# vibevoice-community/VibeVoice

Hardware: AMD Instinct MI355X
Metric: audio-sec/wall-sec (higher is better)
Workload: dtype bf16

## Files before the change

### vibevoice_amd/csrc/block1d.hip

```cpp
#include "vv_common.h"

namespace {

__device__ __forceinline__ float wsum(float v) {
#pragma unroll
    for (int o = 32; o > 0; o >>= 1) v += __shfl_xor(v, o);
    return v;
}
__device__ __forceinline__ float gelu_erf(float u) { return 0.5f * u * (1.0f + erff(u * 0.70710678118654752440f)); }

struct VVBlock {
    const float* xin;
    float* xout;
    float* nst;
    const float *norm_w, *ffn_norm_w, *gamma, *ffn_gamma, *dw_w , *dw_b, *b1, *b2;
    const u32x4 *w1, *w2;
    int T;
    float eps;
    VVSlotIds sl;
    int64_t sx, snst;
};

template <int XS>
__device__ __forceinline__ void split_store(unsigned char* base, size_t part_stride, int byte_off, float v) {
// ... 127 lines not shown
        xs[e] += gam_r * acc;
    }
    __syncthreads();
    for (int r = wave; r < TT; r += 4) {
        float s = 0.f;
        float xr[CL];
#pragma unroll
        for (int q = 0; q < CL; ++q) { const int c = lane + q * 64; xr[q] = (c < C) ? xs[r * C + c] : 0.f; s += xr[q] * xr[q]; }
        const float rr = rsqrtf(wsum(s) / (float)C + a.eps);
#pragma unroll
        for (int q = 0; q < CL; ++q) {
            const int c = lane + q * 64;
            if (c < C) {
                const float n = xr[q] * rr * fnw_r[q];
                const int off = (((c >> 5) * 64 + r + 16 * ((c & 31) >> 3)) * 8 + (c & 7)) * 2;
                split_store<XS>(f1, (size_t)KT1 * 1024, off, n);
            }
        }
    }
    __syncthreads();
#pragma unroll
    for (int i1 = 0; i1 < M1; ++i1) {
        const int nt = wave + 4 * i1;
        if (nt >= NT1) break;
        f32x4 acc = {0.f, 0.f, 0.f, 0.f};
#pragma unroll
        for (int kt = 0; kt < KT1; ++kt) {
            const bf16x8 wf = __builtin_bit_cast(bf16x8, w1r[i1][kt]);
#pragma unroll
            for (int p = 0; p < XS; ++p) {
                const bf16x8 xb = __builtin_bit_cast(bf16x8, *reinterpret_cast<const u32x4*>(f1 + ((size_t)(p * KT1 + kt) * 64 + lane) * 16));
                acc = __builtin_amdgcn_mfma_f32_16x16x32_bf16(wf, xb, acc, 0, 0, 0);
            }
        }
        const int n0 = nt * 16 + fq * 4;
        float u[4];
        const float bb[4] = {b1_r[i1].x, b1_r[i1].y, b1_r[i1].z, b1_r[i1].w};
#pragma unroll
        for (int r = 0; r < 4; ++r) u[r] = gelu_erf(acc[r] + bb[r]);
        const int off = (((n0 >> 5) * 64 + frow + 16 * ((n0 & 31) >> 3)) * 8 + (n0 & 7)) * 2;
#pragma unroll
        for (int r = 0; r < 4; ++r) split_store<XS>(f2, (size_t)KT2 * 1024, off + r * 2, u[r]);
    }
    __syncthreads();
#pragma unroll
    for (int i2 = 0; i2 < M2; ++i2) {
        const int nt = wave + 4 * i2;
        if (nt >= NT2) break;
        f32x4 acc = {0.f, 0.f, 0.f, 0.f};
#pragma unroll
        for (int kt = 0; kt < KT2; ++kt) {
            const bf16x8 wf = __builtin_bit_cast(bf16x8, w2r[i2][kt]);
#pragma unroll
            for (int p = 0; p < XS; ++p) {
                const bf16x8 ub = __builtin_bit_cast(bf16x8, *reinterpret_cast<const u32x4*>(f2 + ((size_t)(p * KT2 + kt) * 64 + lane) * 16));
                acc = __builtin_amdgcn_mfma_f32_16x16x32_bf16(wf, ub, acc, 0, 0, 0);
            }
        }
        const int c0 = nt * 16 + fq * 4;
        const int t = t0 + frow;
        if (t < a.T) {
            float4 o;
            o.x = xs[frow * C + c0 + 0] + fg_r[i2].x * (acc[0] + b2_r[i2].x);
            o.y = xs[frow * C + c0 + 1] + fg_r[i2].y * (acc[1] + b2_r[i2].y);
            o.z = xs[frow * C + c0 + 2] + fg_r[i2].z * (acc[2] + b2_r[i2].z);
            o.w = xs[frow * C + c0 + 3] + fg_r[i2].w * (acc[3] + b2_r[i2].w);
            *reinterpret_cast<float4*>(xout + (int64_t)t * C + c0) = o;
        }
    }
}

template <int C, int XS>
static void go(const VVBlock& a, hipStream_t s) {
    constexpr int TT = 16, HALO = 6, F = 4 * C;
    const size_t smem = (size_t)((TT + HALO) * C + TT * C + TT) * 4 + (size_t)XS * (C / 32) * 1024 + (size_t)XS * (F / 32) * 1024;
    static bool attr = false;
    if (!attr) {
        hipFuncSetAttribute(reinterpret_cast<const void*>(&vv_block1d_kernel<C, XS>), hipFuncAttributeMaxDynamicSharedMemorySize, 160 * 1024);
        attr = true;
    }
    hipLaunchKernelGGL((vv_block1d_kernel<C, XS>), dim3((a.T + TT - 1) / TT, a.sl.n > 0 ? a.sl.n : 1), dim3(256), smem, s, a);
}

}

extern "C" int vv_block1d_supported(int C) { return C == 32 || C == 64 || C == 128; }
extern "C" int vv_block1d_slots_launch(int C, int xs, const float* xin, float* xout, float* nst, const float* norm_w,
                                       const float* ffn_norm_w, const float* gamma, const float* ffn_gamma,
                                       const float* dw_w, const float* dw_b, const float* b1, const float* b2,
                                       const void* w1, const void* w2, int T, float eps, const int* ids, int n, int64_t sx,
                                       int64_t snst, hipStream_t s);

extern "C" int vv_block1d_launch(int C, int xs, const float* xin, float* xout, float* nst, const float* norm_w,
                                 const float* ffn_norm_w, const float* gamma, const float* ffn_gamma,
                                 const float* dw_w, const float* dw_b, const float* b1, const float* b2,
                                 const void* w1, const void* w2, int T, float eps, hipStream_t s) {
    return vv_block1d_slots_launch(C, xs, xin, xout, nst, norm_w, ffn_norm_w, gamma, ffn_gamma, dw_w, dw_b, b1, b2, w1, w2, T, eps,
                                   nullptr, 0, 0, 0, s);
}

extern "C" int vv_block1d_slots_launch(int C, int xs, const float* xin, float* xout, float* nst, const float* norm_w,
                                       const float* ffn_norm_w, const float* gamma, const float* ffn_gamma,
                                       const float* dw_w, const float* dw_b, const float* b1, const float* b2,
                                       const void* w1, const void* w2, int T, float eps, const int* ids, int n, int64_t sx,
                                       int64_t snst, hipStream_t s) {
    if (n < 0 || n > 8) return -1;
    VVBlock a{xin, xout, nst, norm_w, ffn_norm_w, gamma, ffn_gamma, dw_w, dw_b, b1, b2,
              (const u32x4*)w1, (const u32x4*)w2, T, eps};
    a.sl.n = ids ? n : 0;
    for (int i = 0; i < 8; ++i) a.sl.id[i] = (ids && i < n) ? ids[i] : 0;
    a.sx = sx; a.snst = snst;
#define VV_B(C_)                                                     \
    do {                                                             \
        if (xs == 1) go<C_, 1>(a, s);                                \
        else if (xs == 2) go<C_, 2>(a, s);                           \
        else go<C_, 3>(a, s);                                        \
    } while (0)
    if (C == 32) VV_B(32);
    else if (C == 64) VV_B(64);
    else if (C == 128) VV_B(128);
    else return -1;
#undef VV_B
    return vv_launch_rc(0);
}
```

### vibevoice_amd/csrc/engine.hip

```cpp
#include <algorithm>
#include <cmath>
#include <cstdarg>
#include <cstdio>
#include <cstdlib>
#include <cstring>
#include <functional>
#include <map>
#include <set>
#include <string>
#include <vector>

#include <mutex>
#include <shared_mutex>
#include "../../include/vvhip.h"
#include "vv_common.h"

extern "C" {
int vv_gemm_launch(VVGemm a, int xs, hipStream_t s);
int vv_pack_launch(const void* src, int src_is_bf16, void* dst, int N, int K, int kind, int Cin, int Cout, int ksz,
                   int stride, hipStream_t s);
int vv_rope_append_launch(int D, const float* qkv, const VVRow* rows, const float* inv_freq, float* q_out, void* kc,
                          void* vc, int R, int Hq, int Hkv, int64_t cache_stride, int64_t head_stride, hipStream_t s);
int vv_rope_table_launch(const float* inv_freq, void* tab, int n_pos, int half, hipStream_t s);
int vv_attn_fused_launch(int D, int xs, const float* qkv, const VVRow* rows, const void* rope_tab, void* kc, void* vc,
                         int R, int Hq, int Hkv, int64_t cache_stride, int64_t head_stride, int S,
                         float* pm, float* pl, float* po, float* out, void* out_packed, hipStream_t s);
int vv_attn_launch(int D, int xs, const float* q, const VVRow* rows, const void* kc, const void* vc, int R, int Hq,
                   int Hkv, int64_t cache_stride, int64_t head_stride, int S, float* pm, float* pl, float* po,
                   float* out, hipStream_t s);
int vv_embed_launch(const void* table, const int* ids, float* out, int n, int H, hipStream_t s);
int vv_logits_full_launch(const void* table, const float* hidden, float* out, int n, int V, int H, hipStream_t s);
int vv_rmsnorm_rows_launch(const float* x, int ldx, float* y, int ldy, const float* w, int T, int C, float eps, hipStream_t s);
int vv_dwconv_res_launch(const float* nb, const float* x, float* xo, const float* w, const float* b, const float* gamma, int T, int C, hipStream_t s);
int vv_normdw_sliced_ok(int T, int C);
int vv_normdw_sliced_launch(const float* xin, float* xout, float* nb, const float* nw, const float* w, const float* b,
                            const float* gamma, int T, int C, float eps, hipStream_t s);
int vv_normdw_sliced_slots_launch(const float* xin, float* xout, float* nb, const float* nw, const float* w, const float* b,
                                  const float* gamma, int T, int C, float eps, const int* ids, int n, int64_t sx, int64_t snb,
                                  hipStream_t s);
int vv_normdw_rows_slots_launch(const float* xin, float* xout, float* nb, const float* nw, const float* w, const float* b,
                                const float* gamma, int T, int C, float eps, const int* ids, int n, int64_t sx, int64_t snb,
                                hipStream_t s);
int vv_stem_conv_slots_launch(const float* in, const void* wp, const float* bias, float* out, int T, int N, const int* ids, int n,
                              int64_t s_in, int64_t s_out, hipStream_t s);
int vv_head_conv1_slots_launch(const float* x, const void* wp, const float* bias, float* out, int T, int Cin, const int* ids, int n,
                               int64_t s_in, int64_t s_out, hipStream_t s);
int vv_block1d_slots_launch(int C, int xs, const float* xin, float* xout, float* nst, const float* norm_w,
                            const float* ffn_norm_w, const float* gamma, const float* ffn_gamma,
                            const float* dw_w, const float* dw_b, const float* b1, const float* b2,
                            const void* w1, const void* w2, int T, float eps, const int* ids, int n, int64_t sx,
                            int64_t snst, hipStream_t s);
int vv_affine_slots_launch(const float* x, float* y, float mul, float add, int L, const int* ids, int n, int64_t stride, hipStream_t s);
int vv_normdw_launch(float* x, float* nb, const float* nw, const float* w, const float* b, const float* gamma, int T, int C,
                     float eps, hipStream_t s);
int vv_normdw_rows_ok(int T, int C);
int vv_normdw_rows_launch(const float* xin, float* xout, float* nb, const float* nw, const float* w, const float* b,
                          const float* gamma, int T, int C, float eps, hipStream_t s);
int vv_stem_conv_launch(const float* in, const void* wp, const float* bias, float* out, int T, int N, hipStream_t s);
int vv_head_conv1_launch(const float* x, const void* wp, const float* bias, float* out, int T, int Cin, hipStream_t s);
int vv_shift_rows_launch(const void* tab, int n_entries, int maxC, hipStream_t s);
int vv_zero_hist_launch(const void* tab, int n_entries, hipStream_t s);
int vv_cfg_dpm_launch(const float* eps, float* x, float* x0_prev, const float* coef, float cfg, int n, int L, const float* sde_noise, hipStream_t s);
int vv_affine_launch(const float* x, float* y, float mul, float add, int n, hipStream_t s);
int vv_copy_launch(void* dst, const void* src, size_t bytes, hipStream_t s);
int vv_zero_launch(void* dst, size_t bytes, hipStream_t s);
int vv_sampler_init_launch(const float* noise, float* z, float* x0p, int nL, hipStream_t s);
int vv_add_launch(const float* a, const float* b, float* y, int n, hipStream_t s);
int vv_tfreq_launch(const float* t, float* out, int n, hipStream_t s);
int vv_silu_launch(float* x, int n, hipStream_t s);
int vv_ada_in_launch(const float* cproj, const float* temb, float* out, int rows, int n_steps, int H, hipStream_t s);
int vv_add_rows_launch(const float* x, const float* v, float* y, int n, int C, hipStream_t s);
int vv_relu_launch(float* x, int n, hipStream_t s);
int vv_kv_import_launch(const void* k, const void* v, int src_bf16, void* kc, void* vc, int L, int Hkv, int D, int64_t head_stride, int pos0, hipStream_t s);
int vv_kv_move_launch(void* kc, void* vc, int layers, int Hkv, int D, int64_t layer_stride, int64_t head_stride, int src, int dst, hipStream_t s);
int vv_kv_zero_v_tail_launch(void* vc, const VVRow* rows, int R, int layers, int Hkv, int D, int64_t cache_stride, int64_t layer_stride,
                             int64_t head_stride, int max_ctx, hipStream_t s);
int vv_pcm16_launch(const float* x, short* out, int n, int samples, hipStream_t s);
int vv_cvt_launch(const void* src, void* dst, int64_t n, int to_bf16, hipStream_t s);
int vv_dw_transpose_launch(const float* src, float* dst, int C, hipStream_t s);
int vv_pack_rows_launch(const float* x, int ldx, const float* nw, float eps, void* xp, int T, int K, hipStream_t s);
int vv_unpack_rows_launch(const void* xp, float* x, int T, int K, hipStream_t s);
int vv_pack16_launch(const float* x, int ldx, int mode, const float* nw, float eps, const float* sc, const float* sh, int ld_mod,
                     void* xp, int T, int K, hipStream_t s);
int vv_gemv16p_launch(const void* W, const void* W2, const void* Xp, float* Y, void* Yp, const float* bias, const float* gate,
                      int T, int N, int K, int ldy, int ld_gate, int epi, hipStream_t s);
int vv_gemv16p_launch2(const VVGemv16p* a, int epi, int flags, hipStream_t s);
int vv_head_tail_ok(const VVTail* a);
int vv_head_tail_init();
int vv_head_tail_launch(const VVTail* a, hipStream_t s);
int vv_pack16_tiles_launch(const float* x, int ldx, int64_t stride_outer, int n_inner, int64_t stride_inner, void* xp, int64_t tile_bytes,
                           int T, int K, int n_tiles, hipStream_t s);
int vv_ada_pack_launch(const float* cproj, const float* temb, void* xp, int rows, int n_steps, int H, hipStream_t s);
int vv_gemm3_launch(const void* W, const void* W2, const void* Xp, float* Y, void* Yp, const float* bias, int T, int N, int K,
                    int ldy, int epi, const VVGemmWs* ws, hipStream_t s);
int vv_gemm_qkv_rope_launch(const void* W, const void* Xp, const float* bias, int T, int K, int D, int Hq, int Hkv, const VVRow* rows_dev,
                            const void* rope_tab, float* q_out, void* kc, void* vc, int64_t cache_stride, int64_t head_stride,
                            const VVGemmWs* ws, hipStream_t s);
int vv_attn_prefill4_launch(int D, const float* q, const VVRow* rows, const void* kc, const void* vc, int R, int Hq, int Hkv,
                            int64_t cache_stride, int64_t head_stride, float* out, void* out_packed, hipStream_t s);
int vv_block1d_supported(int C);
int vv_gemv_ok(const VVGemm* a);
int vv_tile_ok(const VVGemm* a, int xs);
int vv_block1d_launch(int C, int xs, const float* xin, float* xout, float* nst, const float* norm_w,
                      const float* ffn_norm_w, const float* gamma, const float* ffn_gamma, const float* dw_w,
                      const float* dw_b, const float* b1, const float* b2, const void* w1, const void* w2, int T,
                      float eps, hipStream_t s);
}

struct VVShiftH { float* buf; int T, hist, C; };

static thread_local char g_err[512] = "";
static std::shared_mutex g_dev_mu;
#define VV_SHARED std::shared_lock<std::shared_mutex> _vv_dev_lk(g_dev_mu)
static std::mutex g_family_mu;

namespace {

enum WKind { W_MAT = 0, W_VEC = 1, W_DW = 2, W_TABLE = 3, W_BIAS_REP = 4 };

struct Weight {
    std::string name;
    int kind = W_VEC;
    int64_t nelem = 0;
    void* dev = nullptr;
    int N = 0, K = 0, pk = 0, Cin = 0, Cout = 0, ksz = 0, stride = 0;
    int rep = 1;
    bool loaded = false;
    bool optional = false;
};

struct Block {
    int C;
    float *norm_w, *ffn_norm_w, *gamma, *ffn_gamma, *dw_w, *dw_b, *b1, *b2;
    void *w1, *w2;
    float* nb;
    float* nst;
    int64_t nb_stride;
};

struct ConvG {
    void* w; float* bias;
    int K, N, ldx;
    int rows_per_frame;
};

struct Stage {
    int C, Tpf;
    int hist;
    float* xs;
    float* xs2;
    float* xfinal;
    bool fused;
    bool pp;
    int64_t sl_stride;
    std::vector<Block> blocks;
    ConvG in;
};

struct CodecNet {
    bool decoder = false;
    int Fmax = 1, in_dim = 1, out_dim = 1, in_hist = 6, in_Tpf = 1;
    std::vector<float*> in_buf;
    std::vector<std::vector<Stage>> st;
    ConvG head;
    std::vector<float*> u;
    std::vector<std::map<int, void*>> shift_tab;
    std::vector<int> shift_n;
    std::vector<void*> zero_tab;
    int maxC = 1;
    int kd = 0, ke = 1 << 30;
    bool head_batch = false;
    int64_t in_stride = 0, u_stride = 0;
    std::map<uint64_t, std::pair<void*, int>> shift_multi;
};

struct GraphEntry { hipGraphExec_t exec; uint64_t last_use; };

}

struct vv_ctx {
    vv_config c;
    char err[512];
    std::vector<Weight> w;
// ... 366 lines not shown
    *tab_out = d; *n_out = (int)t.size();
    return 0;
}
static int codec_tables(vv_ctx* ctx, CodecNet& net, int sl, int F, void** tab_out, int* n_out) {
    auto it = net.shift_tab[sl].find(F);
    if (it != net.shift_tab[sl].end()) { *tab_out = it->second; *n_out = net.shift_n[sl]; return 0; }
    std::vector<VVShiftH> t;
    codec_table_entries(net, sl, F, t);
    void* d = dalloc(ctx, t.size() * sizeof(VVShiftH), false);
    if (!d) return -1;
    HIPCHK(ctx, hipMemcpy(d, t.data(), t.size() * sizeof(VVShiftH), hipMemcpyHostToDevice));
    net.shift_tab[sl][F] = d; net.shift_n[sl] = (int)t.size();
    *tab_out = d; *n_out = (int)t.size();
    return 0;
}

static VVGemm mk_gemm(const void* W, const float* X, float* Y, int T, int N, int K, int ldx, int ldy) {
    VVGemm g; memset(&g, 0, sizeof(g));
    g.W = (const u32x4*)W; g.X = X; g.Y = Y; g.T = T; g.N = N; g.K = K; g.ldx = ldx; g.ldy = ldy;
    g.pro = VV_PRO_NONE; g.epi = VV_EPI_STORE; g.ksplit = 0; g.nt = 0; g.eps = 1e-6f;
    return g;
}
static int ksplit_parts(const vv_ctx* ctx, VVGemm& g, float* parts, int part_stride) {
    const int n_tiles = (g.N + 15) / 16, k_tiles = (g.K + 31) / 32;
    constexpr int max_tiles = 128;
    if (g.T > 4 || n_tiles > max_tiles || k_tiles < 96) return 0;
    const int ks = 3;
    g.kgrid = ks; g.yparts = parts; g.part_stride = part_stride;
    if (!vv_gemv_ok(&g)) { g.kgrid = 0; g.yparts = nullptr; g.part_stride = 0; return 0; }
    return ks - 1;
}
static double gemm_bytes(const VVGemm& g) {
    double w = (double)vv_packed_elems(g.N, g.K) * 2.0 * (g.W2 ? 2.0 : 1.0);
    double x = (double)g.T * g.K * 4.0;
    double y = (double)g.T * g.N * 4.0 * ((g.epi == VV_EPI_RESID || g.epi == VV_EPI_GATED_RESID) ? 2.0 : 1.0);
    return w + x + y;
}
static int gemm_prof(vv_ctx* ctx, const VVGemm& g, hipStream_t st) {
    if ((size_t)(2 * ctx->prof_n + 2) > ctx->prof_ev.size()) {
        size_t old = ctx->prof_ev.size();
        ctx->prof_ev.resize(old + 2048);
        for (size_t i = old; i < ctx->prof_ev.size(); ++i) hipEventCreate(&ctx->prof_ev[i]);
    }
    ctx->prof_stream = st;
    hipEventRecord(ctx->prof_ev[2 * ctx->prof_n], st);
    int r = vv_gemm_launch(g, ctx->c.xsplit, st);
    hipEventRecord(ctx->prof_ev[2 * ctx->prof_n + 1], st);
    ctx->prof_n++;
    ctx->prof_bytes += gemm_bytes(g);
    const bool is_gemv = !vv_tile_ok(&g, ctx->c.xsplit) && g.ksplit <= 0 && vv_gemv_ok(&g) && (g.T <= 4 || ctx->c.xsplit <= 2);
    ctx->prof_rec.push_back({g.T, g.N, g.K, g.pro, g.epi, g.W2 ? 1 : 0, gemm_bytes(g), is_gemv});
    if (is_gemv) { ctx->prof_gemv.push_back(g); ctx->prof_gemv_bytes += gemm_bytes(g); }
    return r;
}
#ifdef VV_GEMM_TIMING
constexpr int TL_MAX = 4096, TL_STRIDE = 16 + 2 * 3200;
static int gemm_tl(vv_ctx* ctx, VVGemm g, hipStream_t st) {
    if (!ctx->tl_base && getenv("VVHIP_TIMELINE")) {
        if (hipMalloc(&ctx->tl_base, (size_t)TL_MAX * TL_STRIDE * 8) != hipSuccess) return -9;
        hipMemset(ctx->tl_base, 0, (size_t)TL_MAX * TL_STRIDE * 8);
    }
    const bool gv = vv_gemv_ok(&g) && (g.T <= 4 || ctx->c.xsplit <= 2);
    const bool want = gv ? ((g.T <= 4 || g.T != 16 || g.N > 16384) && (g.N + 15) / 16 <= 3200) : (g.T > 16);
    if (ctx->tl_base && ctx->tl_idx < TL_MAX && want) {
        g.dbg = ctx->tl_base + (size_t)ctx->tl_idx * TL_STRIDE;
        ctx->tl_rec.push_back({g.T, g.N, g.K, g.pro, gv ? g.epi : g.epi + 100});
        ctx->tl_idx++;
    }
    return vv_gemm_launch(g, ctx->c.xsplit, st);
}
extern "C" int vv_timeline_dump(vv_ctx* ctx, unsigned long long* out_host, int* meta_host, int max_launches) {
    VV_SHARED;
    hipDeviceSynchronize();
    const int n = std::min(max_launches, ctx->tl_idx);
    if (n > 0) hipMemcpy(out_host, ctx->tl_base, (size_t)n * TL_STRIDE * 8, hipMemcpyDeviceToHost);
    for (int i = 0; i < n; ++i) { const auto& r = ctx->tl_rec[i]; int* m = meta_host + 5 * i; m[0] = r.T; m[1] = r.N; m[2] = r.K; m[3] = r.pro; m[4] = r.epi; }
    return n;
}
#define GEMM(g) do { ctx->launches++; VVCHK(gemm_tl(ctx, g, st)); } while (0)
#else
#define GEMM(g) do { ctx->launches++; if (ctx->prof_on) VVCHK(gemm_prof(ctx, g, st)); else VVCHK(vv_gemm_launch(g, ctx->c.xsplit, st)); } while (0)
#endif

static int run_codec(vv_ctx* ctx, CodecNet& net, int sl, int F, float* out, hipStream_t st, int i0 = 0, int i1 = -1,
                     bool head = true, bool shift = true, int tail_valid = -1) {
    const float eps = ctx->c.codec_eps;
    const bool stream_w = (F == 1);
    auto& stages = net.st[sl];
    const int ns = (int)stages.size();
    if (i1 < 0) i1 = ns;
    for (int i = i0; i < i1; ++i) {
        Stage& s = stages[i];
        const int T = s.Tpf * F;
        float* x = s.xs + (size_t)s.hist * s.C;
        if (tail_valid >= 0 && i > 0) {
            Stage& pv = stages[i - 1];
            const int Tp = pv.Tpf * F;
            if (tail_valid < Tp)
                VVCHK(vv_zero_launch(pv.xfinal + ((size_t)pv.hist + tail_valid) * pv.C, (size_t)(Tp - tail_valid) * pv.C * 4, st));
            const int r = pv.Tpf / s.Tpf;
            tail_valid = (tail_valid + r - 1) / r;
        }
        {
            const ConvG& cg = s.in;
            const float* X = (i == 0) ? net.in_buf[sl] : stages[i - 1].xfinal;
            const int Trows = cg.rows_per_frame * F;
            if (i == 0 && cg.K == 7 && cg.ldx == 1) {
                ctx->launches++;
                VVCHK(vv_stem_conv_launch(X, cg.w, cg.bias, x, Trows, cg.N, st));
            } else {
                VVGemm g = mk_gemm(cg.w, X, x, Trows, cg.N, cg.K, cg.ldx, cg.N);
                g.epi = VV_EPI_BIAS; g.bias = cg.bias; g.nt = stream_w && Trows <= 16;
                GEMM(g);
            }
        }
        if (s.fused) {
            float* cur = s.xs;
            float* oth = s.xs2;
            for (auto& b : s.blocks) {
                ctx->launches++;
                VVCHK(vv_block1d_launch(s.C, ctx->c.xsplit, cur + (size_t)s.hist * s.C, oth + (size_t)s.hist * s.C, b.nst,
                                        b.norm_w, b.ffn_norm_w, b.gamma, b.ffn_gamma, b.dw_w, b.dw_b, b.b1, b.b2, b.w1, b.w2,
                                        T, eps, st));
                std::swap(cur, oth);
            }
            continue;
        }
        float* xo = s.pp ? s.xs2 + (size_t)s.hist * s.C : x;
        for (auto& b : s.blocks) {
            if (s.pp && T == 1 && vv_normdw_sliced_ok(T, s.C)) {
                VVGemm g1 = mk_gemm(b.w1, x, net.u[sl], T, 4 * s.C, s.C, s.C, 4 * s.C);
                g1.pro = VV_PRO_NORMDW; g1.nw = b.ffn_norm_w; g1.eps = eps; g1.epi = VV_EPI_BIAS_GELU; g1.bias = b.b1; g1.nt = stream_w;
                g1.dw_hist = b.nb; g1.dw_w = b.dw_w; g1.dw_b = b.dw_b; g1.dw_gamma = b.gamma; g1.dw_nw = b.norm_w;
                g1.dw_xout = xo; g1.dw_hnew = b.nb + 6 * (size_t)s.C;
                if (vv_gemv_ok(&g1)) {
                    GEMM(g1);
                    VVGemm g2 = mk_gemm(b.w2, net.u[sl], xo, T, s.C, 4 * s.C, 4 * s.C, s.C);
                    g2.epi = VV_EPI_RESID; g2.bias = b.b2; g2.nscale = b.ffn_gamma; g2.nt = stream_w;
                    GEMM(g2);
                    std::swap(x, xo);
                    continue;
                }
            }
            if (s.pp && vv_normdw_sliced_ok(T, s.C)) {
                ctx->launches += 1;
                VVCHK(vv_normdw_sliced_launch(x, xo, b.nb, b.norm_w, b.dw_w, b.dw_b, b.gamma, T, s.C, eps, st));
            } else if (s.pp && vv_normdw_rows_ok(T, s.C)) {
                ctx->launches += 1;
                VVCHK(vv_normdw_rows_launch(x, xo, b.nb, b.norm_w, b.dw_w, b.dw_b, b.gamma, T, s.C, eps, st));
            } else if (!s.pp && (size_t)T * s.C <= 8192 && (s.C & 3) == 0) {
                ctx->launches += 1;
                VVCHK(vv_normdw_launch(x, b.nb, b.norm_w, b.dw_w, b.dw_b, b.gamma, T, s.C, eps, st));
            } else {
                ctx->launches += 2;
                VVCHK(vv_rmsnorm_rows_launch(x, s.C, b.nb + 6 * (size_t)s.C, s.C, b.norm_w, T, s.C, eps, st));
                VVCHK(vv_dwconv_res_launch(b.nb, x, xo, b.dw_w, b.dw_b, b.gamma, T, s.C, st));
            }
            VVGemm g1 = mk_gemm(b.w1, xo, net.u[sl], T, 4 * s.C, s.C, s.C, 4 * s.C);
            g1.pro = VV_PRO_RMS; g1.nw = b.ffn_norm_w; g1.eps = eps; g1.epi = VV_EPI_BIAS_GELU; g1.bias = b.b1;
            g1.nt = stream_w && T <= 16;
            GEMM(g1);
            VVGemm g2 = mk_gemm(b.w2, net.u[sl], xo, T, s.C, 4 * s.C, 4 * s.C, s.C);
            g2.epi = VV_EPI_RESID; g2.bias = b.b2; g2.nscale = b.ffn_gamma; g2.nt = stream_w && T <= 16;
            GEMM(g2);
            if (s.pp) std::swap(x, xo);
        }
    }
    if (head) {
        const ConvG& cg = net.head;
        Stage& s = stages[ns - 1];
        if (cg.N == 1 && cg.K == 7 * cg.ldx && (cg.ldx & 3) == 0 && cg.ldx <= 1024) {
            ctx->launches++;
            VVCHK(vv_head_conv1_launch(s.xfinal, cg.w, cg.bias, out, cg.rows_per_frame * F, cg.ldx, st));
        } else {
            VVGemm g = mk_gemm(cg.w, s.xfinal, out, cg.rows_per_frame * F, cg.N, cg.K, cg.ldx, cg.N);
            g.epi = VV_EPI_BIAS; g.bias = cg.bias;
            GEMM(g);
        }
    }
    if (!shift) return 0;
    void* tab; int nt;
    if (codec_tables(ctx, net, sl, F, &tab, &nt)) return -1;
    ctx->launches++;
    VVCHK(vv_shift_rows_launch(tab, nt, net.maxC, st));
    return 0;
}

static int run_codec_batch(vv_ctx* ctx, CodecNet& net, const int* ids, int n, int i0, int i1, float* out, bool head, hipStream_t st) {
    const float eps = ctx->c.codec_eps;
    auto& st0 = net.st[0];
    const int ns = (int)st0.size();
    auto slots = [&](VVGemm& g, int T, int64_t sx, int64_t sy) {
        g.sl_n = n; g.sl_T = T; g.sl_x = (int)sx; g.sl_y = (int)sy; g.T = n * T;
        for (int j = 0; j < 8; ++j) g.sl_id[j] = j < n ? ids[j] : 0;
    };
    for (int i = i0; i < i1; ++i) {
        Stage& s = st0[i];
        const int T = s.Tpf;
        float* x = s.xs + (size_t)s.hist * s.C;
        {
            const ConvG& cg = s.in;
            const float* X = (i == 0) ? net.in_buf[0] : st0[i - 1].xfinal;
            const int64_t sx = (i == 0) ? net.in_stride : st0[i - 1].sl_stride;
            if (i == 0 && cg.K == 7 && cg.ldx == 1) {
                ctx->launches++;
                VVCHK(vv_stem_conv_slots_launch(X, cg.w, cg.bias, x, cg.rows_per_frame, cg.N, ids, n, sx, s.sl_stride, st));
            } else {
                VVGemm g = mk_gemm(cg.w, X, x, cg.rows_per_frame, cg.N, cg.K, cg.ldx, cg.N);
                g.epi = VV_EPI_BIAS; g.bias = cg.bias; g.nt = 1;
                slots(g, cg.rows_per_frame, sx, s.sl_stride);
                GEMM(g);
            }
        }
        float* xo = s.xs2 + (size_t)s.hist * s.C;
        if (s.fused) {
            for (auto& b : s.blocks) {
                ctx->launches++;
                VVCHK(vv_block1d_slots_launch(s.C, ctx->c.xsplit, x, xo, b.nst, b.norm_w, b.ffn_norm_w, b.gamma, b.ffn_gamma, b.dw_w, b.dw_b,
                                              b.b1, b.b2, b.w1, b.w2, T, eps, ids, n, s.sl_stride, b.nb_stride, st));
                std::swap(x, xo);
            }
            continue;
        }
        for (auto& b : s.blocks) {
            ctx->launches += 1;
            if (vv_normdw_sliced_ok(T, s.C))
                VVCHK(vv_normdw_sliced_slots_launch(x, xo, b.nb, b.norm_w, b.dw_w, b.dw_b, b.gamma, T, s.C, eps, ids, n, s.sl_stride, b.nb_stride, st));
            else
                VVCHK(vv_normdw_rows_slots_launch(x, xo, b.nb, b.norm_w, b.dw_w, b.dw_b, b.gamma, T, s.C, eps, ids, n, s.sl_stride, b.nb_stride, st));
            VVGemm g1 = mk_gemm(b.w1, xo, net.u[0], T, 4 * s.C, s.C, s.C, 4 * s.C);
            g1.pro = VV_PRO_RMS; g1.nw = b.ffn_norm_w; g1.eps = eps; g1.epi = VV_EPI_BIAS_GELU; g1.bias = b.b1; g1.nt = 1;
            slots(g1, T, s.sl_stride, 0);
            GEMM(g1);
            VVGemm g2 = mk_gemm(b.w2, net.u[0], xo, T, s.C, 4 * s.C, 4 * s.C, s.C);
            g2.epi = VV_EPI_RESID; g2.bias = b.b2; g2.nscale = b.ffn_gamma; g2.nt = 1;
            slots(g2, T, 0, s.sl_stride);
            GEMM(g2);
            std::swap(x, xo);
        }
    }
    if (head) {
        const ConvG& cg = net.head;
        Stage& s = st0[ns - 1];
        if (cg.N == 1 && cg.K == 7 * cg.ldx && (cg.ldx & 3) == 0 && cg.ldx <= 1024) {
            ctx->launches++;
            VVCHK(vv_head_conv1_slots_launch(s.xfinal, cg.w, cg.bias, out, cg.rows_per_frame, cg.ldx, ids, n, s.sl_stride, cg.rows_per_frame, st));
        } else {
            VVGemm g = mk_gemm(cg.w, s.xfinal, out, cg.rows_per_frame, cg.N, cg.K, cg.ldx, cg.N);
            g.epi = VV_EPI_BIAS; g.bias = cg.bias;
            slots(g, cg.rows_per_frame, s.sl_stride, 0);
            GEMM(g);
        }
    }
    return 0;
}

static int zero_codec(vv_ctx* ctx, CodecNet& net, int sl, hipStream_t st) {
    void* tab; int nt;
    if (codec_tables(ctx, net, sl, 1, &tab, &nt)) return -1;
    ctx->launches++;
    VVCHK(vv_zero_hist_launch(tab, nt, st));
    return 0;
}

template <class F>
static int graphed(vv_ctx* ctx, const std::string& key, hipStream_t st, F&& body) {
    if (!ctx->c.use_graph || ctx->prof_on) { VV_SHARED; return body(); }
    auto it = ctx->graphs.find(key);
    if (it == ctx->graphs.end()) {
        if (ctx->seen.size() > 8192) ctx->seen.clear();
        if (ctx->seen.insert(key).second) { VV_SHARED; return body(); }
        hipGraph_t graph = nullptr;
        GraphEntry ge; ge.last_use = 0;
        bool captured = false;
        {
            std::unique_lock<std::shared_mutex> lk(g_dev_mu);
            HIPCHK(ctx, hipStreamBeginCapture(st, hipStreamCaptureModeRelaxed));
            const int r = body();
            const hipError_t e = hipStreamEndCapture(st, &graph);
            if (r == 0 && e == hipSuccess) {
                size_t nn = 0;
                if (hipGraphGetNodes(graph, nullptr, &nn) == hipSuccess && nn) {
                    std::vector<hipGraphNode_t> nodes(nn);
                    if (hipGraphGetNodes(graph, nodes.data(), &nn) == hipSuccess)
                        for (size_t i = 0; i < nn; ++i) { hipGraphNodeType t; if (hipGraphNodeGetType(nodes[i], &t) == hipSuccess && t != hipGraphNodeTypeKernel) ctx->foreign_nodes++; }
                }
                HIPCHK(ctx, hipGraphInstantiate(&ge.exec, graph, nullptr, nullptr, 0));
                hipGraphDestroy(graph);
                captured = true;
            } else {
                (void)hipGetLastError();
                ctx->capture_fallbacks++;
                snprintf(ctx->last_capture_issue, sizeof(ctx->last_capture_issue), "capture of '%s': body rc %d, hipStreamEndCapture: %s", key.c_str(), r, hipGetErrorString(e));
            }
        }
        if (!captured) {
            VV_SHARED;
// ... 1230 lines not shown
```

### vibevoice_amd/csrc/vv_common.h

```cpp
#pragma once
#include <hip/hip_runtime.h>
#include <stdint.h>

typedef __attribute__((ext_vector_type(8))) __bf16 bf16x8;
typedef __attribute__((ext_vector_type(2))) __bf16 bf16x2;
typedef __attribute__((ext_vector_type(4))) float f32x4;
typedef __attribute__((ext_vector_type(2))) float f32x2;
typedef __attribute__((ext_vector_type(4))) unsigned int u32x4;

#define VV_WAVE 64

static inline __host__ __device__ int64_t vv_packed_elems(int N, int K) {
    return (int64_t)((N + 15) / 16) * ((K + 31) / 32) * 512;
}

struct VVRow {
    int cache;
    int pos;
};

struct VVGemmWs {
    float* partials;
    unsigned* flags;
    unsigned* err;
// ... 13 lines not shown
    const float* X;
    float* Y;
    const float* nw;
    const float* mod_scale;
    const float* mod_shift;
    const float* addvec;
    const float* bias;
    const float* nscale;
    const float* gate;
    int T, N, K;
    int ldx, ldy, ld_mod, ld_gate;
    int pro, epi;
    int ksplit;
    int nt;
    int t_pad;
    float* z;
    float* x0p;
    const float* coef;
    float cfg;
    int n_cfg;
    const float* sde_noise;
    unsigned long long* dbg;
    int x_row_mod, add_rows_per_vec;
    float eps;
    int kgrid;
    float* yparts;
    const float* xa;
    const float* ya;
    int n_xa, n_ya;
    int part_stride;
    int sl_n, sl_T, sl_x, sl_y;
    int sl_id[8];
    const float* dw_hist;
    const float* dw_w;
    const float* dw_b;
    const float* dw_gamma;
    const float* dw_nw;
    float* dw_xout;
    float* dw_hnew;
};

struct VVGemv16p {
    const u32x4* W;
    const u32x4* W2;
    const u32x4* Xp;
    float* Y;
    unsigned char* Yp;
    const float* bias;
    const float* gate;
    int T, N, K, ldy, ld_gate;
    const float* ssq_in;
    int ssq_tiles;
    float eps;
    const u32x4* Xs;
    const float* pk_nw;
    const float* pk_sc;
    int ld_pk;
    float* ssq_out;
    float* z; float* x0p; const float* coef; float cfg; int n_cfg; const float* sde_noise;
};

struct VVTail {
    const u32x4* Wout;
    const u32x4* Win;
    const float* bin;
    const float* X;
    const float* xa; int n_xa, part_stride;
    const float* sc; const float* sh; int ld_mod;
    float* Xout;
    const float* z_in; const float* x0p_in;
    float* z_out; float* x0p_out;
    const float* coef; float cfg; int n_cfg; const float* sde_noise;
    int T, H, L; float eps;
};

struct VVSlotIds { int n; int id[8]; };
__device__ __forceinline__ int vv_slot_id(const int (&id)[8], int j) {
    int r = id[0];
#pragma unroll
    for (int i = 1; i < 8; ++i) r = (j == i) ? id[i] : r;
    return r;
}

inline thread_local int g_vv_launch_err = 0;
static inline int vv_launch_rc(int rc_ok) {
    const hipError_t e = hipGetLastError();
    if (e == hipSuccess) return rc_ok;
    g_vv_launch_err = (int)e;
    return -2;
}
```

Before: 16.49.

## Fuse three consecutive codec conv blocks into one stage kernel with halo recompute

Adds a stage-level kernel that runs all three ConvNeXt-style 1D blocks of a codec stage (RMSNorm, 7-tap depthwise conv, RMSNorm+FFN with MFMA, residuals) in a single launch. Each workgroup loads an extended halo of input rows into shared memory and recomputes the overlapping rows, so intermediate activations never go back to global memory. For small channel counts all three blocks' weights are preloaded into registers. The intent is to remove two of the three launches per stage and their global round-trips. The cost is redundant halo computation, higher register and shared-memory pressure, and smaller time tiles for C=128.

```diff
diff --git a/vibevoice_amd/csrc/block1d.hip b/vibevoice_amd/csrc/block1d.hip
--- a/vibevoice_amd/csrc/block1d.hip
+++ b/vibevoice_amd/csrc/block1d.hip
@@ -233,6 +233,251 @@
     hipLaunchKernelGGL((vv_block1d_kernel<C, XS>), dim3((a.T + TT - 1) / TT, a.sl.n > 0 ? a.sl.n : 1), dim3(256), smem, s, a);
 }
 
+constexpr int stage_rows(int TO) {
+    int m = 0;
+    for (int b = 0; b < 3; ++b) {
+        const int n = TO + 6 * (2 - b), r = 6 * (b + 1) + (n + 15) / 16 * 16;
+        m = r > m ? r : m;
+    }
+    return m;
+}
+
+template <int C, int XS, int TO>
+__global__ __launch_bounds__(256) void vv_stage1d_kernel(const VVStage a) {
+    constexpr int NB = 3, HALO = 6, F = 4 * C;
+    constexpr int KT1 = C / 32, NT1 = F / 16;
+    constexpr int KT2 = F / 32, NT2 = C / 16;
+    constexpr int LO0 = HALO * NB;
+    constexpr int NRL = LO0 + TO;
+    constexpr int XR = stage_rows(TO);
+    constexpr bool PRE = C <= 64;
+    constexpr int NW = PRE ? NB : 1;
+    extern __shared__ __attribute__((aligned(16))) unsigned char smem[];
+    float* X = reinterpret_cast<float*>(smem);
+    float* nrm = X + XR * C;
+    unsigned char* f1 = reinterpret_cast<unsigned char*>(nrm + XR * C);
+    unsigned char* f2 = f1 + (size_t)XS * KT1 * 1024;
+    const int tid = threadIdx.x, lane = tid & 63;
+    const int wave = __builtin_amdgcn_readfirstlane(tid >> 6);
+    const int t0 = blockIdx.x * TO;
+    const float* xin = a.xin; float* xout = a.xout;
+    int64_t nst_off = 0;
+    if (a.sl.n > 0) {
+        const int64_t id = vv_slot_id(a.sl.id, blockIdx.y);
+        xin += id * a.sx; xout += id * a.sx; nst_off = id * a.snst;
+    }
+    constexpr int M1 = (NT1 + 3) / 4, M2 = (NT2 + 3) / 4;
+    u32x4 w1r[NW][M1][KT1], w2r[NW][M2][KT2];
+    auto load_w = [&](const int slot, const VVStageBlk& p) __attribute__((always_inline)) {
+#pragma unroll
+        for (int i = 0; i < M1; ++i) {
+            const int nt = wave + 4 * i;
+#pragma unroll
+            for (int kt = 0; kt < KT1; ++kt)
+                w1r[slot][i][kt] = (nt < NT1) ? p.w1[((int64_t)nt * KT1 + kt) * 64 + lane] : u32x4{0u, 0u, 0u, 0u};
+        }
+#pragma unroll
+        for (int i = 0; i < M2; ++i) {
+            const int nt = wave + 4 * i;
+#pragma unroll
+            for (int kt = 0; kt < KT2; ++kt)
+                w2r[slot][i][kt] = (nt < NT2) ? p.w2[((int64_t)nt * KT2 + kt) * 64 + lane] : u32x4{0u, 0u, 0u, 0u};
+        }
+    };
+    if constexpr (PRE) {
+#pragma unroll
+        for (int b = 0; b < NB; ++b) load_w(b, a.b[b]);
+    } else {
+        load_w(0, a.b[0]);
+    }
+    for (int e = tid * 4; e < XR * C; e += 1024) {
+        const int r = e / C, c = e % C;
+        const int t = t0 - LO0 + r;
+        float4 v = {0.f, 0.f, 0.f, 0.f};
+        if (r < NRL && t >= 0 && t < a.T) v = *reinterpret_cast<const float4*>(xin + (int64_t)t * C + c);
+        *reinterpret_cast<float4*>(X + e) = v;
+    }
+    constexpr int CL = (C + 63) / 64;
+    const int cc = tid % C;
+    const int frow = lane & 15, fq = lane >> 4;
+#pragma unroll
+    for (int b = 0; b < NB; ++b) {
+        const VVStageBlk& p = a.b[b];
+        const int RB = HALO * (b + 1);
+        const int NR = TO + HALO * (NB - 1 - b);
+        const int wb = PRE ? b : 0;
+        if constexpr (!PRE) { if (b > 0) load_w(0, p); }
+        float* nst = p.nst + nst_off;
+        float nw_r[CL], fnw_r[CL];
+#pragma unroll
+        for (int i = 0; i < CL; ++i) {
+            const int c = lane + i * 64;
+            nw_r[i] = (c < C) ? p.norm_w[c] : 0.f;
+            fnw_r[i] = (c < C) ? p.ffn_norm_w[c] : 0.f;
+        }
+        float dw_r[7];
+#pragma unroll
+        for (int j = 0; j < 7; ++j) dw_r[j] = p.dw_w[j * C + cc];
+        const float dwb_r = p.dw_b[cc], gam_r = p.gamma[cc];
+        float4 b1_r[M1], b2_r[M2], fg_r[M2];
+#pragma unroll
+        for (int i = 0; i < M1; ++i) {
+            const int nt = wave + 4 * i;
+            b1_r[i] = (nt < NT1) ? *reinterpret_cast<const float4*>(p.b1 + nt * 16 + fq * 4) : float4{0.f, 0.f, 0.f, 0.f};
+        }
+#pragma unroll
+        for (int i = 0; i < M2; ++i) {
+            const int nt = wave + 4 * i;
+            b2_r[i] = (nt < NT2) ? *reinterpret_cast<const float4*>(p.b2 + nt * 16 + fq * 4) : float4{0.f, 0.f, 0.f, 0.f};
+            fg_r[i] = (nt < NT2) ? *reinterpret_cast<const float4*>(p.ffn_gamma + nt * 16 + fq * 4) : float4{0.f, 0.f, 0.f, 0.f};
+        }
+        __syncthreads();
+        for (int rr = wave; rr < NR + HALO; rr += 4) {
+            const int r = RB - HALO + rr;
+            const int t = t0 - LO0 + r;
+            if (t < 0) {
+#pragma unroll
+                for (int q = 0; q < CL; ++q) {
+                    const int c = lane + q * 64;
+                    if (c < C) nrm[r * C + c] = (t >= -HALO) ? nst[(HALO + t) * C + c] : 0.f;
+                }
+            } else if (t < a.T) {
+                float xv[CL];
+                float s = 0.f;
+#pragma unroll
+                for (int q = 0; q < CL; ++q) { const int c = lane + q * 64; xv[q] = (c < C) ? X[r * C + c] : 0.f; }
+#pragma unroll
+                for (int q = 0; q < CL; ++q) s += xv[q] * xv[q];
+                const float rs = rsqrtf(wsum(s) / (float)C + a.eps);
+#pragma unroll
+                for (int q = 0; q < CL; ++q) {
+                    const int c = lane + q * 64;
+                    if (c < C) {
+                        const float n = xv[q] * rs * nw_r[q];
+                        nrm[r * C + c] = n;
+                        if (t >= a.T - HALO && t >= t0) nst[(HALO + t - (a.T - HALO)) * C + c] = n;
+                    }
+                }
+            } else {
+#pragma unroll
+                for (int q = 0; q < CL; ++q) { const int c = lane + q * 64; if (c < C) nrm[r * C + c] = 0.f; }
+            }
+        }
+        __syncthreads();
+        for (int e = tid; e < NR * C; e += 256) {
+            const int r = RB - HALO + e / C;
+            float acc = dwb_r;
+#pragma unroll
+            for (int j = 0; j < 7; ++j) acc += dw_r[j] * nrm[(r + j) * C + cc];
+            X[RB * C + e] += gam_r * acc;
+        }
+        __syncthreads();
+        for (int r0 = RB; r0 < RB + NR; r0 += 16) {
+            for (int r = wave; r < 16; r += 4) {
+                float s = 0.f;
+                float xr[CL];
+#pragma unroll
+                for (int q = 0; q < CL; ++q) { const int c = lane + q * 64; xr[q] = (c < C) ? X[(r0 + r) * C + c] : 0.f; s += xr[q] * xr[q]; }
+                const float rr = rsqrtf(wsum(s) / (float)C + a.eps);
+#pragma unroll
+                for (int q = 0; q < CL; ++q) {
+                    const int c = lane + q * 64;
+                    if (c < C) {
+                        const float n = xr[q] * rr * fnw_r[q];
+                        const int off = (((c >> 5) * 64 + r + 16 * ((c & 31) >> 3)) * 8 + (c & 7)) * 2;
+                        split_store<XS>(f1, (size_t)KT1 * 1024, off, n);
+                    }
+                }
+            }
+            __syncthreads();
+#pragma unroll
+            for (int i1 = 0; i1 < M1; ++i1) {
+                const int nt = wave + 4 * i1;
+                if (nt >= NT1) break;
+                f32x4 acc = {0.f, 0.f, 0.f, 0.f};
+#pragma unroll
+                for (int kt = 0; kt < KT1; ++kt) {
+                    const bf16x8 wf = __builtin_bit_cast(bf16x8, w1r[wb][i1][kt]);
+#pragma unroll
+                    for (int q = 0; q < XS; ++q) {
+                        const bf16x8 xb = __builtin_bit_cast(bf16x8, *reinterpret_cast<const u32x4*>(f1 + ((size_t)(q * KT1 + kt) * 64 + lane) * 16));
+                        acc = __builtin_amdgcn_mfma_f32_16x16x32_bf16(wf, xb, acc, 0, 0, 0);
+                    }
+                }
+                const int n0 = nt * 16 + fq * 4;
+                float u[4];
+                const float bb[4] = {b1_r[i1].x, b1_r[i1].y, b1_r[i1].z, b1_r[i1].w};
+#pragma unroll
+                for (int r = 0; r < 4; ++r) u[r] = gelu_erf(acc[r] + bb[r]);
+                const int off = (((n0 >> 5) * 64 + frow + 16 * ((n0 & 31) >> 3)) * 8 + (n0 & 7)) * 2;
+#pragma unroll
+                for (int r = 0; r < 4; ++r) split_store<XS>(f2, (size_t)KT2 * 1024, off + r * 2, u[r]);
+            }
+            __syncthreads();
+#pragma unroll
+            for (int i2 = 0; i2 < M2; ++i2) {
+                const int nt = wave + 4 * i2;
+                if (nt >= NT2) break;
+                f32x4 acc = {0.f, 0.f, 0.f, 0.f};
+#pragma unroll
+                for (int kt = 0; kt < KT2; ++kt) {
+                    const bf16x8 wf = __builtin_bit_cast(bf16x8, w2r[wb][i2][kt]);
+#pragma unroll
+                    for (int q = 0; q < XS; ++q) {
+                        const bf16x8 ub = __builtin_bit_cast(bf16x8, *reinterpret_cast<const u32x4*>(f2 + ((size_t)(q * KT2 + kt) * 64 + lane) * 16));
+                        acc = __builtin_amdgcn_mfma_f32_16x16x32_bf16(wf, ub, acc, 0, 0, 0);
+                    }
+                }
+                const int c0 = nt * 16 + fq * 4;
+                const int r = r0 + frow;
+                const int t = t0 - LO0 + r;
+                if (r < RB + NR && t >= 0 && t < a.T) {
+                    float* xr = X + r * C + c0;
+                    float4 o;
+                    o.x = xr[0] + fg_r[i2].x * (acc[0] + b2_r[i2].x);
+                    o.y = xr[1] + fg_r[i2].y * (acc[1] + b2_r[i2].y);
+                    o.z = xr[2] + fg_r[i2].z * (acc[2] + b2_r[i2].z);
+                    o.w = xr[3] + fg_r[i2].w * (acc[3] + b2_r[i2].w);
+                    if (b == NB - 1) *reinterpret_cast<float4*>(xout + (int64_t)t * C + c0) = o;
+                    else *reinterpret_cast<float4*>(xr) = o;
+                }
+            }
+        }
+    }
+}
+
+template <int C, int XS, int TO>
+static void go_stage(const VVStage& a, hipStream_t s) {
+    constexpr int XR = stage_rows(TO), F = 4 * C;
+    const size_t smem = (size_t)2 * XR * C * 4 + (size_t)XS * (C / 32) * 1024 + (size_t)XS * (F / 32) * 1024;
+    static bool attr = false;
+    if (!attr) {
+        hipFuncSetAttribute(reinterpret_cast<const void*>(&vv_stage1d_kernel<C, XS, TO>), hipFuncAttributeMaxDynamicSharedMemorySize, 160 * 1024);
+        attr = true;
+    }
+    hipLaunchKernelGGL((vv_stage1d_kernel<C, XS, TO>), dim3((a.T + TO - 1) / TO, a.sl.n > 0 ? a.sl.n : 1), dim3(256), smem, s, a);
+}
+
+}
+
+extern "C" int vv_stage1d_ok(int C, int n_blocks, int T) { return (C == 32 || C == 64 || C == 128) && n_blocks == 3 && T >= 8; }
+extern "C" int vv_stage1d_launch(const VVStage* st, int C, int xs, const int* ids, int n, hipStream_t s) {
+    if (n < 0 || n > 8 || st->xin == st->xout) return -1;
+    VVStage a = *st;
+    a.sl.n = ids ? n : 0;
+    for (int i = 0; i < 8; ++i) a.sl.id[i] = (ids && i < n) ? ids[i] : 0;
+#define VV_S(C_, TO_)                                                \
+    do {                                                             \
+        if (xs == 1) go_stage<C_, 1, TO_>(a, s);                     \
+        else if (xs == 2) go_stage<C_, 2, TO_>(a, s);                \
+        else go_stage<C_, 3, TO_>(a, s);                             \
+    } while (0)
+    if (C == 32) VV_S(32, 10);
+    else if (C == 64) VV_S(64, 10);
+    else if (C == 128) VV_S(128, 4);
+    else return -1;
+#undef VV_S
+    return vv_launch_rc(0);
 }
 
 extern "C" int vv_block1d_supported(int C) { return C == 32 || C == 64 || C == 128; }
diff --git a/vibevoice_amd/csrc/engine.hip b/vibevoice_amd/csrc/engine.hip
--- a/vibevoice_amd/csrc/engine.hip
+++ b/vibevoice_amd/csrc/engine.hip
@@ -99,6 +99,8 @@
 int vv_attn_prefill4_launch(int D, const float* q, const VVRow* rows, const void* kc, const void* vc, int R, int Hq, int Hkv,
                             int64_t cache_stride, int64_t head_stride, float* out, void* out_packed, hipStream_t s);
 int vv_block1d_supported(int C);
+int vv_stage1d_ok(int C, int n_blocks, int T);
+int vv_stage1d_launch(const VVStage* st, int C, int xs, const int* ids, int n, hipStream_t s);
 int vv_gemv_ok(const VVGemm* a);
 int vv_tile_ok(const VVGemm* a, int xs);
 int vv_block1d_launch(int C, int xs, const float* xin, float* xout, float* nst, const float* norm_w,
@@ -631,6 +633,22 @@
 #define GEMM(g) do { ctx->launches++; if (ctx->prof_on) VVCHK(gemm_prof(ctx, g, st)); else VVCHK(vv_gemm_launch(g, ctx->c.xsplit, st)); } while (0)
 #endif
 
+static bool stage1d_ok(const Stage& s, int T) {
+    return s.fused && vv_stage1d_ok(s.C, (int)s.blocks.size(), T) && s.xfinal != s.xs;
+}
+static int stage1d(vv_ctx* ctx, Stage& s, int T, float eps, const int* ids, int n, hipStream_t st) {
+    VVStage a; memset(&a, 0, sizeof(a));
+    a.xin = s.xs + (size_t)s.hist * s.C; a.xout = s.xfinal + (size_t)s.hist * s.C;
+    for (int j = 0; j < 3; ++j) {
+        const Block& b = s.blocks[j];
+        a.b[j] = {b.nst, b.norm_w, b.ffn_norm_w, b.gamma, b.ffn_gamma, b.dw_w, b.dw_b, b.b1, b.b2, (const u32x4*)b.w1, (const u32x4*)b.w2};
+    }
+    a.T = T; a.eps = eps; a.sx = s.sl_stride; a.snst = s.blocks[0].nb_stride;
+    ctx->launches++;
+    VVCHK(vv_stage1d_launch(&a, s.C, ctx->c.xsplit, ids, n, st));
+    return 0;
+}
+
 static int run_codec(vv_ctx* ctx, CodecNet& net, int sl, int F, float* out, hipStream_t st, int i0 = 0, int i1 = -1,
                      bool head = true, bool shift = true, int tail_valid = -1) {
     const float eps = ctx->c.codec_eps;
@@ -662,6 +680,10 @@
                 g.epi = VV_EPI_BIAS; g.bias = cg.bias; g.nt = stream_w && Trows <= 16;
                 GEMM(g);
             }
+        }
+        if (F == 1 && stage1d_ok(s, T)) {
+            if (stage1d(ctx, s, T, eps, nullptr, 0, st)) return -1;
+            continue;
         }
         if (s.fused) {
             float* cur = s.xs;
@@ -762,6 +784,10 @@
             }
         }
         float* xo = s.xs2 + (size_t)s.hist * s.C;
+        if (stage1d_ok(s, T)) {
+            if (stage1d(ctx, s, T, eps, ids, n, st)) return -1;
+            continue;
+        }
         if (s.fused) {
             for (auto& b : s.blocks) {
                 ctx->launches++;
diff --git a/vibevoice_amd/csrc/vv_common.h b/vibevoice_amd/csrc/vv_common.h
--- a/vibevoice_amd/csrc/vv_common.h
+++ b/vibevoice_amd/csrc/vv_common.h
@@ -119,6 +119,21 @@
     return r;
 }
 
+struct VVStageBlk {
+    float* nst;
+    const float *norm_w, *ffn_norm_w, *gamma, *ffn_gamma, *dw_w , *dw_b, *b1, *b2;
+    const u32x4 *w1, *w2;
+};
+struct VVStage {
+    const float* xin;
+    float* xout;
+    VVStageBlk b[3];
+    int T;
+    float eps;
+    VVSlotIds sl;
+    int64_t sx, snst;
+};
+
 inline thread_local int g_vv_launch_err = 0;
 static inline int vv_launch_rc(int rc_ok) {
     const hipError_t e = hipGetLastError();
```

Result: no change. 16.56, median of 6 (+0.4%).
